# magenta/ddsp

Measured on NVIDIA H100. Metric: audio samples/sec (Harmonic+FilteredNoise decoder), higher is better.
Workload: dtype f32

## Files before the change

### ddsp_b200/csrc/harmonic_v4.cuh

```cuda
#pragma once
#include "harmonic_common.cuh"

namespace ddsp {

__device__ __noinline__ float harmonic_sample_exact(const float* x0,
                                                    const float* x1, float w0,
                                                    float w1, uint32_t p32,
                                                    float f_lo, float f_hi,
                                                    float frac, int K,
                                                    float nyq) {
  float acc = 0.f;
  uint32_t pk = 0;
  for (int k = 1; k <= K; ++k) {
    pk += p32;
    if (!(ref_harmonic_freq(f_lo, f_hi, frac, k) < nyq)) continue;
    float a = x0[k - 1] * w0 + x1[k - 1] * w1;
    acc = fmaf(a, sinpif((float)(int)pk * 4.656612873077393e-10f), acc);
  }
  return acc;
}

namespace hv4 {

constexpr int NW = 4;
constexpr int NT = NW * 32;
constexpr int MIN_CTAS = 6;

#ifdef DDSP_HV4_TIMING
constexpr int kTimingPhases = 8;
__device__ unsigned long long g_hv4_timing[kMaxSMs * (kTimingPhases + 1)];
#define HV4_TIMING_DECL                                                                 \
  unsigned tacc__[kTimingPhases] = {0, 0, 0, 0, 0, 0, 0, 0};                            \
  unsigned tprev__ = (unsigned)clock()
#define HV4_LAP(i)                                                                      \
  do {                                                                                  \
    const unsigned n__ = (unsigned)clock();                                             \
    tacc__[i] += n__ - tprev__;                                                         \
    tprev__ = n__;                                                                      \
  } while (0)
#define HV4_TIMING_FLUSH()                                                              \
  do {                                                                                  \
    if (lane == 0) {                                                                    \
      unsigned smid__;                                                                  \
      asm volatile("mov.u32 %0, %%smid;" : "=r"(smid__));                               \
      unsigned long long* t__ = g_hv4_timing + (smid__ % kMaxSMs) * (kTimingPhases + 1); \
      for (int i__ = 0; i__ < kTimingPhases; ++i__) atomicAdd(t__ + i__, (unsigned long long)tacc__[i__]); \
      atomicAdd(t__ + kTimingPhases, 1ull);                                             \
    }                                                                                   \
  } while (0)
#else
#define HV4_TIMING_DECL
#define HV4_LAP(i)
#define HV4_TIMING_FLUSH()
#endif

struct __align__(16) FrameRec {
  unsigned long long P, A;
  unsigned long long D;
  int ng;
  int rem;
  float f_lo, f_hi, amp0, amp1;
};
static_assert(sizeof(FrameRec) == 48, "FrameRec must be three 16-byte words");

struct Smem {
  size_t off_mbar, off_sin, off_cos, off_x, off_w, off_red, off_inv, off_rec, off_live, total;
};

__host__ __device__ inline Smem smem_layout(int FW, int Kp, int hop) {
  Smem s;
  const size_t FT = (size_t)FW * NW;
  size_t o = 0;
  s.off_mbar = o; o += 16;
  s.off_sin = o;  o += sizeof(float) * kSinTab;
  s.off_cos = o;  o += sizeof(float) * kSinTab;
  s.off_x = o;    o += sizeof(float) * (FT + 1) * Kp;
  s.off_w = o;    o += (hop == 64) ? 0 : sizeof(float) * hop;
  o = (o + 15) & ~(size_t)15;
  s.off_red = o;  o += 16 * NW;
  s.off_rec = o;  o += sizeof(FrameRec) * FT;
  s.off_inv = o;  o += sizeof(float) * (FT + 1);
  s.off_live = o; o += sizeof(int) * (FT + 1);
  s.total = (o + 15) & ~(size_t)15;
  return s;
}

using hcm::phase32;

__device__ __forceinline__ float4 lds128(uint32_t a) {
  float4 v;
  asm volatile("ld.shared.v4.f32 {%0, %1, %2, %3}, [%4];"
               : "=f"(v.x), "=f"(v.y), "=f"(v.z), "=f"(v.w)
               : "r"(a));
  return v;
}

__device__ __forceinline__ float2 bffma2(float x, float2 v, float2 acc) {
  return ffma2(make_float2(x, x), v, acc);
}
__device__ __forceinline__ float2 bfmul2(float x, float2 v) {
  return fmul2(make_float2(x, x), v);
}

__device__ __forceinline__ void controls_rows4(float* __restrict__ sXw,
                                               const int* __restrict__ sLive,
                                               float* __restrict__ sInv, int r0,
                                               int nrows, int Kp, bool raw_scale,
                                               int lane) {
  const int K4 = Kp >> 2;
  const int sub = lane >> 3, l8 = lane & 7;
  const int r = r0 + sub;
  const bool row_ok = r < nrows;
  float4* row4 = reinterpret_cast<float4*>(sXw + (row_ok ? r : r0) * Kp);
  const int live = row_ok ? sLive[r] : 0;
  const int live4 = (live + 3) >> 2;
  float sum = 0.f;
  int c4 = l8;
  for (; c4 < live4; c4 += 8) {
    float4 x = row4[c4];
    if (raw_scale) {
      x.x = exp_sigmoid_f(x.x); x.y = exp_sigmoid_f(x.y);
      x.z = exp_sigmoid_f(x.z); x.w = exp_sigmoid_f(x.w);
    }
    const int k = 4 * c4;
    if (k + 1 >= live) x.y = 0.f;
    if (k + 2 >= live) x.z = 0.f;
    if (k + 3 >= live) x.w = 0.f;
    sum += (x.x + x.y) + (x.z + x.w);
    row4[c4] = x;
  }
  if (row_ok) {
    const float4 z = make_float4(0.f, 0.f, 0.f, 0.f);
    for (; c4 < K4; c4 += 8) row4[c4] = z;
  }
  sum += __shfl_xor_sync(0xffffffffu, sum, 4);
  sum += __shfl_xor_sync(0xffffffffu, sum, 2);
  sum += __shfl_xor_sync(0xffffffffu, sum, 1);
  if (row_ok && l8 == 0) sInv[r] = __fdividef(1.0f, (sum == 0.0f) ? 1e-7f : sum);
}

__device__ __forceinline__ void controls_rows(float* __restrict__ sXw,
                                              const int* __restrict__ sLive, int r0,
                                              int nrows, int Kp, bool raw_scale,
                                              int lane) {
  const int K4 = Kp >> 2;
  const int sub = lane >> 3, l8 = lane & 7;
  const int r = r0 + sub;
  const bool row_ok = r < nrows;
  float4* row4 = reinterpret_cast<float4*>(sXw + (row_ok ? r : r0) * Kp);
  const int live = sLive[row_ok ? r : r0];
  float sum = 0.f;
  if (row_ok) {
    for (int c4 = l8; c4 < K4; c4 += 8) {
      float4 v = make_float4(0.f, 0.f, 0.f, 0.f);
      if (4 * c4 < live) {
        v = row4[c4];
        float e[4] = {v.x, v.y, v.z, v.w};
#pragma unroll
        for (int u = 0; u < 4; ++u) {
          float w = e[u];
          if (raw_scale) w = exp_sigmoid_f(w);
          if (4 * c4 + u >= live) w = 0.f;
          e[u] = w;
          sum += w;
        }
        v = make_float4(e[0], e[1], e[2], e[3]);
      }
      row4[c4] = v;
    }
  }
  sum += __shfl_xor_sync(0xffffffffu, sum, 4);
  sum += __shfl_xor_sync(0xffffffffu, sum, 2);
  sum += __shfl_xor_sync(0xffffffffu, sum, 1);
  const float inv = 1.0f / ((sum == 0.0f) ? 1e-7f : sum);
  if (row_ok) {
    for (int c4 = l8; 4 * c4 < live; c4 += 8) {
      float4 v = row4[c4];
      v.x *= inv; v.y *= inv; v.z *= inv; v.w *= inv;
      row4[c4] = v;
    }
  }
}

__device__ __forceinline__ int row_live_count(float fq, int K, float nyquist, bool nyq) {
  int live = K;
  if (nyq && fq > 0.f) {
    int k = (int)fminf(nyquist / fq, (float)K);
    while (k < K && __fmul_rn(fq, (float)(k + 1)) < nyquist) ++k;
    while (k > 0 && !(__fmul_rn(fq, (float)k) < nyquist)) --k;
    live = k;
  }
  return live;
}

__device__ __noinline__ float sample_exact(const float* x0, int row_stride, float w0,
                                           float w1, uint32_t p32, float f_lo, float f_hi,
                                           float frac, int K, float nyq) {
  return harmonic_sample_exact(x0, x0 + row_stride, w0, w1, p32, f_lo, f_hi, frac, K, nyq);
}

struct Osc2 {
  float2 vo, ve, dlo, dle, na, sg;
  float2 s0e, s0o, s1e, s1o;
  float2 t0e, t0o, t1e, t1o;
};

__device__ __forceinline__ void osc_seed2(Osc2& st, uint32_t qa, uint32_t qb,
                                          const float* __restrict__ sSin,
                                          const float* __restrict__ sCos) {
  const uint32_t ia = qa >> (32 - kSinTabBits), ib = qb >> (32 - kSinTabBits);
  const float2 tx = make_float2(sSin[ia], sSin[ib]);
  const float2 ty = make_float2(sCos[ia], sCos[ib]);
  constexpr uint32_t kLow = (1u << (32 - kSinTabBits)) - 1u;
  constexpr float kC = 1.4629180792671596e-9f;
  constexpr float kOff = -(float)(1u << (31 - kSinTabBits)) * kC;
  const float2 eps = ffma2(make_float2((float)(qa & kLow), (float)(qb & kLow)),
                                make_float2(kC, kC), make_float2(kOff, kOff));
  const float2 e2 = fmul2(eps, eps);
  const float2 ce = ffma2(e2, make_float2(-0.5f, -0.5f), make_float2(1.f, 1.f));
  const float2 se = fmul2(eps, ffma2(e2, make_float2(-0.16666667f, -0.16666667f),
                                               make_float2(1.f, 1.f)));
  const float2 nse = make_float2(-se.x, -se.y);
  const float2 s1 = ffma2(ty, se, fmul2(tx, ce));
  const float2 c1 = ffma2(tx, nse, fmul2(ty, ce));
  const float2 ss = fmul2(s1, s1), cc = fmul2(c1, c1);
  const float2 s2 = fmul2(fadd2(s1, s1), c1);
  st.sg = make_float2(ss.x > cc.x ? -1.0f : 1.0f, ss.y > cc.y ? -1.0f : 1.0f);
  st.na = fmul2(make_float2(fminf(ss.x, cc.x), fminf(ss.y, cc.y)),
                     make_float2(-4.0f, -4.0f));
  st.vo = s1;
  st.ve = s2;
  st.dlo = ffma2(s1, st.sg, s1);
  st.dle = s2;
}

__device__ __forceinline__ void osc_step(Osc2& st) {
  st.dlo = ffma2(st.na, st.vo, st.dlo);
  st.dle = ffma2(st.na, st.ve, st.dle);
  st.vo = fadd2(st.vo, st.dlo);
  st.ve = fadd2(st.ve, st.dle);
}

__device__ __forceinline__ void osc_group(Osc2& st, const float4& X0, const float4& X1) {
  st.s0e = bffma2(X0.x, st.vo, st.s0e);
  st.s1e = bffma2(X1.x, st.vo, st.s1e);
  st.t0e = bffma2(X0.y, st.ve, st.t0e);
  st.t1e = bffma2(X1.y, st.ve, st.t1e);
  osc_step(st);
  st.s0o = bffma2(X0.z, st.vo, st.s0o);
  st.s1o = bffma2(X1.z, st.vo, st.s1o);
  st.t0o = bffma2(X0.w, st.ve, st.t0o);
  st.t1o = bffma2(X1.w, st.ve, st.t1o);
  osc_step(st);
}

__device__ __forceinline__ void osc_group_first(Osc2& st, const float4& X0,
                                                const float4& X1) {
  st.s0e = bfmul2(X0.x, st.vo);
  st.s1e = bfmul2(X1.x, st.vo);
  st.t0e = bfmul2(X0.y, st.ve);
  st.t1e = bfmul2(X1.y, st.ve);
  osc_step(st);
  st.s0o = bfmul2(X0.z, st.vo);
  st.s1o = bfmul2(X1.z, st.vo);
  st.t0o = bfmul2(X0.w, st.ve);
  st.t1o = bfmul2(X1.w, st.ve);
  osc_step(st);
}

__device__ __forceinline__ void osc_group_masked(Osc2& st, const float4& X0,
                                                 const float4& X1, int k, int ka,
                                                 int kb) {
  float2 mo = make_float2(k + 1 <= ka ? st.vo.x : 0.f, k + 1 <= kb ? st.vo.y : 0.f);
  float2 me = make_float2(k + 2 <= ka ? st.ve.x : 0.f, k + 2 <= kb ? st.ve.y : 0.f);
  st.s0e = bffma2(X0.x, mo, st.s0e);
  st.s1e = bffma2(X1.x, mo, st.s1e);
  st.t0e = bffma2(X0.y, me, st.t0e);
  st.t1e = bffma2(X1.y, me, st.t1e);
  osc_step(st);
  mo = make_float2(k + 3 <= ka ? st.vo.x : 0.f, k + 3 <= kb ? st.vo.y : 0.f);
  me = make_float2(k + 4 <= ka ? st.ve.x : 0.f, k + 4 <= kb ? st.ve.y : 0.f);
  st.s0o = bffma2(X0.z, mo, st.s0o);
  st.s1o = bffma2(X1.z, mo, st.s1o);
  st.t0o = bffma2(X0.w, me, st.t0o);
  st.t1o = bffma2(X1.w, me, st.t1o);
  osc_step(st);
}

__device__ __forceinline__ float4 mask4u(const float4& X, int rem) {
  return make_float4(X.x, rem > 1 ? X.y : 0.f, rem > 2 ? X.z : 0.f, 0.f);
}

struct LaneConst {
  uint32_t c1a, c2a, c1b, c2b;
  float2 w1;
};

template <bool WINDOW>
__device__ __forceinline__ LaneConst lane_const(int r0, int lane, float inv_hop,
                                                const float* __restrict__ sW) {
  LaneConst c;
  const uint32_t ra = r0 + lane, rb = ra + 32;
  c.c1a = ra + 1; c.c2a = (ra * (ra + 1)) >> 1;
  c.c1b = rb + 1; c.c2b = (rb * (rb + 1)) >> 1;
  asm volatile("" : "+r"(c.c1a), "+r"(c.c2a), "+r"(c.c1b), "+r"(c.c2b));
  if (sW != nullptr) {
    c.w1 = make_float2(sW[ra], sW[rb]);
  } else {
    const float fa = (float)ra * inv_hop, fb = (float)rb * inv_hop;
    c.w1 = make_float2(WINDOW ? (0.5f - 0.5f * cospif(fa)) : fa,
                       WINDOW ? (0.5f - 0.5f * cospif(fb)) : fb);
  }
  asm volatile("" : "+f"(c.w1.x), "+f"(c.w1.y));
  return c;
}

__device__ __forceinline__ void frame_chunk(
    const float* __restrict__ sX, int xoff, int Kp, const FrameRec* __restrict__ rec,
    const LaneConst& lc, int r0, float inv_hop, const float* __restrict__ sSin,
    const float* __restrict__ sCos, int K, float nyquist, int lane,
    float* __restrict__ out, int accumulate) {
  const float* __restrict__ x0 = sX + xoff;
  const uint32_t kp4 = (uint32_t)Kp << 2;
  const ulonglong2 PA = *reinterpret_cast<const ulonglong2*>(&rec->P);
  const uint4 Dk = *reinterpret_cast<const uint4*>(&rec->D);
  const float4 fa = *reinterpret_cast<const float4*>(&rec->f_lo);
  const unsigned long long D = ((unsigned long long)Dk.y << 32) | Dk.x;
  const int ng = (int)Dk.z, rem = (int)Dk.w;
  const uint32_t qa = phase32(PA.x, PA.y, D, lc.c1a, lc.c2a);
  const uint32_t qb = phase32(PA.x, PA.y, D, lc.c1b, lc.c2b);
  const float2 w0 = ffma2(make_float2(-lc.w1.x, -lc.w1.y), make_float2(fa.z, fa.z),
                               make_float2(fa.z, fa.z));
  const float2 w1 = bfmul2(fa.w, lc.w1);
  float2 y;
  if (ng < 0) {
    constexpr uint32_t kRound = 1u << (31 - kSinTabBits);
    int ra = r0 + lane, xo = xoff;
    asm volatile("" : "+r"(ra), "+r"(xo));
    const float fra = (float)ra * inv_hop, frb = (float)(ra + 32) * inv_hop;
    y.x = sample_exact(sX + xo, Kp, w0.x, w1.x, qa - kRound, fa.x, fa.y, fra, K, nyquist);
    y.y = sample_exact(sX + xo, Kp, w0.y, w1.y, qb - kRound, fa.x, fa.y, frb, K, nyquist);
  } else {
    Osc2 st;
    osc_seed2(st, qa, qb, sSin, sCos);
    if (ng > 0) {
      uint32_t a = smem_u32(x0);
      const uint32_t a_end = a + (ng << 4);
      osc_group_first(st, lds128(a), lds128(a + kp4));
      a += 16;
      if ((ng & 1) == 0) {
        osc_group(st, lds128(a), lds128(a + kp4));
        a += 16;
      }
#pragma unroll 1
      while (a != a_end) {
        osc_group(st, lds128(a), lds128(a + kp4));
        osc_group(st, lds128(a + 16), lds128(a + kp4 + 16));
        a += 32;
      }
      if (rem != 0) osc_group(st, mask4u(lds128(a), rem), mask4u(lds128(a + kp4), rem));
    } else {
      int ra = r0 + lane;
      asm volatile("" : "+r"(ra));
      const float fra = (float)ra * inv_hop, frb = (float)(ra + 32) * inv_hop;
      const int ka = live_harmonics(fa.x, fa.y, fra, K, nyquist);
      const int kb = live_harmonics(fa.x, fa.y, frb, K, nyquist);
      const int kmin = __reduce_min_sync(0xffffffffu, min(ka, kb));
      const int kmax = __reduce_max_sync(0xffffffffu, max(ka, kb));
      st.s0e = st.s0o = st.s1e = st.s1o = make_float2(0.f, 0.f);
      st.t0e = st.t0o = st.t1e = st.t1o = make_float2(0.f, 0.f);
      uint32_t a = smem_u32(x0);
      const uint32_t a_main = a + ((kmin & ~3) << 2);
      if (kmin & 4) {
        osc_group(st, lds128(a), lds128(a + kp4));
        a += 16;
      }
#pragma unroll 1
      while (a != a_main) {
        osc_group(st, lds128(a), lds128(a + kp4));
        osc_group(st, lds128(a + 16), lds128(a + kp4 + 16));
        a += 32;
      }
      for (int k = kmin & ~3; k < kmax; k += 4, a += 16)
        osc_group_masked(st, lds128(a), lds128(a + kp4), k, ka, kb);
    }
    const float2 t0 = ffma2(st.sg, fadd2(st.s0o, st.t0o), fadd2(st.s0e, st.t0e));
    const float2 t1 = ffma2(st.sg, fadd2(st.s1o, st.t1o), fadd2(st.s1e, st.t1e));
    y = ffma2(t1, w1, fmul2(t0, w0));
  }
  if (accumulate) {
    y.x += out[0];
    y.y += out[32];
  }
  out[0] = y.x;
  out[32] = y.y;
}

template <bool WINDOW, int HOPT>
__global__ void __launch_bounds__(NT, MIN_CTAS)
harmonic_v4_kernel(HarmonicParams p, int use_tma, int FW) {
  extern __shared__ __align__(16) unsigned char smem_raw[];
  const int hop = HOPT ? HOPT : p.hop;
  const int Kp = p.Kp, K = p.K, F = p.F;
  const int FT = FW * NW;
  const Smem L = smem_layout(FW, Kp, hop);
  void* mbar = (void*)(smem_raw + L.off_mbar);
  float* sSin = (float*)(smem_raw + L.off_sin);
  float* sCos = (float*)(smem_raw + L.off_cos);
  float* sX = (float*)(smem_raw + L.off_x);
  float* sW = (HOPT == 64) ? nullptr : (float*)(smem_raw + L.off_w);
  double* sRedD = (double*)(smem_raw + L.off_red);
  unsigned long long* sWarpTot = (unsigned long long*)(smem_raw + L.off_red) + NW;
  float* sInv = (float*)(smem_raw + L.off_inv);
  FrameRec* sRec = (FrameRec*)(smem_raw + L.off_rec);
  int* sLive = (int*)(smem_raw + L.off_live);

  const int b = blockIdx.y;
  const int i0 = blockIdx.x * FT;
  const int nfr = min(FT, F - i0);
  const int rows_in = min(nfr + 1, F - i0);
  const int tid = threadIdx.x, lane = tid & 31, warp = tid >> 5;
  const float* f0b = p.f0 + (size_t)b * F;
  const float* ampb = p.amps + (size_t)b * F;

  asm volatile("griddepcontrol.launch_dependents;" ::: "memory");
  HV4_TIMING_DECL;
  if (use_tma && tid == 0) {
    mbar_init(mbar, 1);
    const uint32_t bytes = (uint32_t)rows_in * (uint32_t)K * 4u;
    mbar_expect_tx(mbar, bytes);
    tma_bulk_g2s(sX, p.hd + ((size_t)b * F + i0) * K, bytes, mbar);
  }

  const int n_rec = (FT + 31) >> 5;
  const bool rec_warp = warp < n_rec;
  const int fr = warp * 32 + lane;
  const int cnt = max(0, min(32, nfr - warp * 32));
  const bool raw_scale = p.ctl_flags & DDSP_B200_CTL_SCALE;
  const int n_ctl = (NW > n_rec) ? NW - n_rec : NW;
  const int cw = (NW > n_rec) ? warp - n_rec : warp;
  const int rw = (nfr + n_ctl - 1) / n_ctl;
  const int c0 = cw * rw;
  const int ncr = (cw < 0) ? 0 : max(0, min(rw, nfr - c0));
  const bool c_last = ncr > 0 && c0 + ncr == nfr;
  const int nrows = ncr + ((c_last && rows_in > nfr) ? 1 : 0);
  const float f_row = (lane < nrows) ? f0b[min(i0 + c0 + lane, F - 1)] : 0.f;
  float f = 0.f, a = 0.f, f_tile = 0.f, f_first = 0.f;
  float f_x = 0.f, a_x = 0.f;
  if (rec_warp && cnt > 0) {
    if (lane <= cnt) {
      const int g = min(i0 + fr, F - 1);
      f = f0b[g];
      a = ampb[g];
    }
    if (lane == 31 && cnt == 32) {
      const int g = min(i0 + fr + 1, F - 1);
      f_x = f0b[g];
      a_x = ampb[g];
    }
    f_tile = f0b[i0];
    f_first = f0b[0];
  }
  constexpr int TPT = kSinTab / NT;
  static_assert(TPT * NT == kSinTab, "the table splits evenly over the CTA");
  float2 tab[TPT];
#pragma unroll
  for (int u = 0; u < TPT; ++u) tab[u] = hcm::g_sincos256[tid + u * NT];
  double part = 0.0;
  if ((reinterpret_cast<uintptr_t>(f0b) & 15) == 0) {
    const float4* f4 = reinterpret_cast<const float4*>(f0b);
    const int n4 = i0 >> 2;
    float4 v[4];
    int j = tid;
    for (; j + 3 * NT < n4; j += 4 * NT) {
#pragma unroll
      for (int u = 0; u < 4; ++u) v[u] = f4[j + u * NT];
#pragma unroll
      for (int u = 0; u < 4; ++u)
        part += ((double)v[u].x + (double)v[u].y) + ((double)v[u].z + (double)v[u].w);
    }
#pragma unroll
    for (int u = 0; u < 4; ++u)
      v[u] = (j + u * NT < n4) ? f4[j + u * NT] : make_float4(0.f, 0.f, 0.f, 0.f);
    const float tail = (tid < (i0 & 3)) ? f0b[4 * n4 + tid] : 0.f;
#pragma unroll
    for (int u = 0; u < 4; ++u)
      part += ((double)v[u].x + (double)v[u].y) + ((double)v[u].z + (double)v[u].w);
    part += (double)tail;
  } else {
#pragma unroll 4
    for (int j = tid; j < i0; j += NT) part += (double)f0b[j];
  }
#pragma unroll
  for (int o = 16; o > 0; o >>= 1) part += __shfl_xor_sync(0xffffffffu, part, o);
  if (lane == 0) sRedD[warp] = part;
#pragma unroll
  for (int u = 0; u < TPT; ++u) {
    sSin[tid + u * NT] = tab[u].x;
    sCos[tid + u * NT] = tab[u].y;
  }
  const float inv_hop = 1.0f / (float)hop;
  if (HOPT != 64) {
    for (int r = tid; r < hop; r += NT) {
      const float frac = (float)r * inv_hop;
      sW[r] = WINDOW ? (0.5f - 0.5f * cospif(frac)) : frac;
    }
  }
  if (!use_tma) {
    if (p.hd != nullptr) {
      const float* hdb = p.hd + ((size_t)b * F + i0) * K;
      for (int idx = tid; idx < rows_in * Kp; idx += NT) {
        int r = idx / Kp, c = idx - r * Kp;
        sX[idx] = (c < K) ? hdb[r * K + c] : 0.f;
      }
    } else {
      for (int idx = tid; idx < rows_in * Kp; idx += NT)
        sX[idx] = (idx % Kp == 0) ? 1.0f : 0.f;
    }
  }
  HV4_LAP(0);
  __syncthreads();
  HV4_LAP(1);

  const bool have_ctl = (p.ctl_flags != 0) && (p.hd != nullptr);
  const bool zero_ok = have_ctl && (p.ctl_flags & DDSP_B200_CTL_NYQUIST);
  unsigned long long excl = 0;
  if (rec_warp && cnt > 0) {
    if (raw_scale && lane <= cnt) a = exp_sigmoid_f(a);
    const float f_next = __shfl_down_sync(0xffffffffu, f, 1);
    const float a_next = __shfl_down_sync(0xffffffffu, a, 1);
    float f_n = f_next, a_n = a_next;
    if (lane == 31 && cnt == 32) {
      f_n = f_x;
      a_n = raw_scale ? exp_sigmoid_f(a_x) : a_x;
    }
    unsigned long long tot = 0;
    double a0 = 0.0, dd = 0.0;
    if (lane < cnt) {
      a0 = (double)f * p.inv_sr;
      const double a1 = (double)f_n * p.inv_sr;
      dd = (a1 - a0) * (1.0 / (double)hop);
      tot = frame_total_fix64(a0, a1, hop);
    }
    const unsigned long long incl = warp_scan_frame_totals(tot, lane);
    excl = incl - tot;
    if (lane == 31) sWarpTot[warp] = incl;
    const bool nyq = p.ctl_flags & DDSP_B200_CTL_NYQUIST;
    const int live = row_live_count(f, K, p.nyquist, nyq);
    int live_next = __shfl_down_sync(0xffffffffu, live, 1);
    if (lane == 31 && cnt == 32) live_next = row_live_count(f_n, K, p.nyquist, nyq);
    int ng = -1, rem = 0;
    if (lane < cnt && f >= 1.0f && f_n >= 1.0f) {
      const int kca = live_harmonics(f, f_n, 0.0f, K, p.nyquist);
      const int kcb = live_harmonics(f, f_n, (float)(hop - 1) * inv_hop, K, p.nyquist);
      ng = 0;
      if (kca == kcb) {
        if (zero_ok && live == kca && live_next <= kca) {
          ng = max(1, (kca + 3) >> 2);
        } else {
          ng = kca >> 2;
          rem = kca & 3;
        }
      }
    }
    if (lane < cnt) {
      FrameRec r;
      r.P = 0; r.A = turns_to_fix64(a0); r.D = turns_to_fix64(dd);
      r.ng = ng; r.rem = rem;
      r.f_lo = f; r.f_hi = f_n; r.amp0 = a; r.amp1 = a_n;
      sRec[fr] = r;
    }
    const int n_act = (nfr + 31) >> 5;
    if (n_act > 1) asm volatile("bar.sync 1, %0;" ::"r"(32 * n_act) : "memory");
    HV4_LAP(2);

    double base_sum = 0.0;
#pragma unroll
    for (int w = 0; w < NW; ++w) base_sum += sRedD[w];
    const double a_tile = (double)f_tile * p.inv_sr;
    const double a_first = (double)f_first * p.inv_sr;
    unsigned long long P0 = tile_phase_base(base_sum, a_first, a_tile, hop, p.inv_sr);
    for (int w = 0; w < warp; ++w) P0 += sWarpTot[w];
    if (lane < cnt) {
      const unsigned long long Pf = P0 + excl;
      sRec[fr].P = Pf + 0x80000000ull + (1ull << (63 - kSinTabBits));
    }
  }
  HV4_LAP(3);

  if (ncr > 0) {
    float* sXw = sX + (size_t)c0 * Kp;
    if (have_ctl) {
      const bool nyq = p.ctl_flags & DDSP_B200_CTL_NYQUIST;
      for (int r = lane; r < nrows; r += 32)
        sLive[c0 + r] = row_live_count(r == lane ? f_row : f0b[min(i0 + c0 + r, F - 1)], K,
                                       p.nyquist, nyq);
      __syncwarp();
    }
    if (use_tma) mbar_wait(mbar, 0);
    HV4_LAP(4);
    if (have_ctl) {
      if (Kp <= 128) {
        for (int r0 = 0; r0 < nrows; r0 += 4)
          controls_rows4(sXw, sLive + c0, sInv + c0, r0, nrows, Kp, raw_scale, lane);
      } else {
        for (int r0 = 0; r0 < nrows; r0 += 4)
          controls_rows(sXw, sLive + c0, r0, nrows, Kp, raw_scale, lane);
        for (int r = lane; r < nrows; r += 32) sInv[c0 + r] = 1.0f;
      }
    } else {
      for (int r = lane; r < nrows; r += 32) sInv[c0 + r] = 1.0f;
    }
    if (c_last && rows_in < nfr + 1) {
      __syncwarp();
      for (int c = lane; c < Kp; c += 32) sXw[ncr * Kp + c] = sXw[(ncr - 1) * Kp + c];
      if (lane == 0) sInv[c0 + ncr] = sInv[c0 + ncr - 1];
    }
  }
  HV4_LAP(5);
  __syncthreads();
  HV4_LAP(6);

  const int w0f = warp * FW;
  const int nfw = max(0, min(FW, nfr - w0f));
  if (nfw > 0) {
    FrameRec* rec = sRec + w0f;
    if (lane < nfw) {
      rec[lane].amp0 *= sInv[w0f + lane];
      rec[lane].amp1 *= sInv[w0f + lane + 1];
    }
    __syncwarp();
    float* o = p.audio + (size_t)b * p.N + (size_t)(i0 + w0f) * hop + lane;
    int xoff = w0f * Kp;
    if (HOPT == 64) {
      const LaneConst lc = lane_const<WINDOW>(0, lane, inv_hop, nullptr);
#pragma unroll 1
      for (int li = 0; li < nfw; ++li, ++rec, xoff += Kp, o += 64) {
        frame_chunk(sX, xoff, Kp, rec, lc, 0, inv_hop, sSin, sCos, K, p.nyquist, lane, o,
                    p.accumulate);
      }
    } else {
      for (int li = 0; li < nfw; ++li, ++rec, xoff += Kp) {
        for (int r0 = 0; r0 < hop; r0 += 64, o += 64) {
          const LaneConst lc = lane_const<WINDOW>(r0, lane, inv_hop, sW);
          frame_chunk(sX, xoff, Kp, rec, lc, r0, inv_hop, sSin, sCos, K, p.nyquist, lane, o,
                      p.accumulate);
        }
      }
    }
  }
  HV4_LAP(7);
  HV4_TIMING_FLUSH();
}

}

inline int launch_harmonic_v4(HarmonicParams p, cudaStream_t st) {
  using namespace hv4;
  p.Kp = (p.K + 3) & ~3;
  int FW = 8;
  const long long want_ctas = 8ll * num_sms();
  while (FW > 4 && (long long)p.B * ((p.F + FW * NW - 1) / (FW * NW)) < want_ctas) FW = (FW + 1) >> 1;
  while (FW > 1 && (long long)p.B * ((p.F + FW * NW - 1) / (FW * NW)) < num_sms()) FW = (FW + 1) >> 1;
  FW =std::max(1, std::min(FW, (p.F + NW - 1) / NW));
  while (FW > 1 && smem_layout(FW, p.Kp, p.hop).total > 64 * 1024) FW = (FW + 1) / 2;
  const size_t smem = smem_layout(FW, p.Kp, p.hop).total;
  if (smem > kMaxDynSmem) return 1;
  const int use_tma = (p.hd != nullptr) && (p.K % 4 == 0) &&
                      (((uintptr_t)p.hd & 15) == 0);
  dim3 grid((p.F + FW * NW - 1) / (FW * NW), p.B);
  const bool win = p.amp_method == DDSP_B200_AMP_WINDOW;
  auto kern = p.hop == 64 ? (win ? harmonic_v4_kernel<true, 64> : harmonic_v4_kernel<false, 64>)
                          : (win ? harmonic_v4_kernel<true, 0> : harmonic_v4_kernel<false, 0>);
  int rc = set_smem(kern, smem, "harmonic_forward(v4)");
  if (rc) return rc;
  kern<<<grid, NT, smem, st>>>(p, use_tma, FW);
  DDSP_CHECK_LAUNCH("harmonic_forward(v4)");
  return 0;
}

}
```

Measured before the change: 48.92 billion.

## Interleave sin/cos table and reuse per-row live counts via named barrier

Merges the separate sin and cos shared-memory tables into one interleaved float2 table, so each oscillator seed does one 64-bit load per index instead of two scalar loads. The record-building warps no longer recompute live harmonic counts with shuffles. They wait on a named barrier for the other warps to fill sLive, then read it. The partial-sum loop also breaks early on out-of-range vector slots. The barrier adds a cross-warp dependency that could stall the record warps, and its arrive/sync counts must match exactly.

```diff
diff --git a/ddsp_b200/csrc/harmonic_v4.cuh b/ddsp_b200/csrc/harmonic_v4.cuh
--- a/ddsp_b200/csrc/harmonic_v4.cuh
+++ b/ddsp_b200/csrc/harmonic_v4.cuh
@@ -64,7 +64,7 @@
 static_assert(sizeof(FrameRec) == 48, "FrameRec must be three 16-byte words");
 
 struct Smem {
-  size_t off_mbar, off_sin, off_cos, off_x, off_w, off_red, off_inv, off_rec, off_live, total;
+  size_t off_mbar, off_tab, off_x, off_w, off_red, off_inv, off_rec, off_live, total;
 };
 
 __host__ __device__ inline Smem smem_layout(int FW, int Kp, int hop) {
@@ -72,8 +72,7 @@
   const size_t FT = (size_t)FW * NW;
   size_t o = 0;
   s.off_mbar = o; o += 16;
-  s.off_sin = o;  o += sizeof(float) * kSinTab;
-  s.off_cos = o;  o += sizeof(float) * kSinTab;
+  s.off_tab = o;  o += sizeof(float2) * kSinTab;
   s.off_x = o;    o += sizeof(float) * (FT + 1) * Kp;
   s.off_w = o;    o += (hop == 64) ? 0 : sizeof(float) * hop;
   o = (o + 15) & ~(size_t)15;
@@ -206,11 +205,11 @@
 };
 
 __device__ __forceinline__ void osc_seed2(Osc2& st, uint32_t qa, uint32_t qb,
-                                          const float* __restrict__ sSin,
-                                          const float* __restrict__ sCos) {
+                                          const float2* __restrict__ sTab) {
   const uint32_t ia = qa >> (32 - kSinTabBits), ib = qb >> (32 - kSinTabBits);
-  const float2 tx = make_float2(sSin[ia], sSin[ib]);
-  const float2 ty = make_float2(sCos[ia], sCos[ib]);
+  const float2 ta = sTab[ia], tb = sTab[ib];
+  const float2 tx = make_float2(ta.x, tb.x);
+  const float2 ty = make_float2(ta.y, tb.y);
   constexpr uint32_t kLow = (1u << (32 - kSinTabBits)) - 1u;
   constexpr float kC = 1.4629180792671596e-9f;
   constexpr float kOff = -(float)(1u << (31 - kSinTabBits)) * kC;
@@ -317,9 +316,8 @@
 
 __device__ __forceinline__ void frame_chunk(
     const float* __restrict__ sX, int xoff, int Kp, const FrameRec* __restrict__ rec,
-    const LaneConst& lc, int r0, float inv_hop, const float* __restrict__ sSin,
-    const float* __restrict__ sCos, int K, float nyquist, int lane,
-    float* __restrict__ out, int accumulate) {
+    const LaneConst& lc, int r0, float inv_hop, const float2* __restrict__ sTab, int K,
+    float nyquist, int lane, float* __restrict__ out, int accumulate) {
   const float* __restrict__ x0 = sX + xoff;
   const uint32_t kp4 = (uint32_t)Kp << 2;
   const ulonglong2 PA = *reinterpret_cast<const ulonglong2*>(&rec->P);
@@ -342,7 +340,7 @@
     y.y = sample_exact(sX + xo, Kp, w0.y, w1.y, qb - kRound, fa.x, fa.y, frb, K, nyquist);
   } else {
     Osc2 st;
-    osc_seed2(st, qa, qb, sSin, sCos);
+    osc_seed2(st, qa, qb, sTab);
     if (ng > 0) {
       uint32_t a = smem_u32(x0);
       const uint32_t a_end = a + (ng << 4);
@@ -405,8 +403,7 @@
   const int FT = FW * NW;
   const Smem L = smem_layout(FW, Kp, hop);
   void* mbar = (void*)(smem_raw + L.off_mbar);
-  float* sSin = (float*)(smem_raw + L.off_sin);
-  float* sCos = (float*)(smem_raw + L.off_cos);
+  float2* sTab = (float2*)(smem_raw + L.off_tab);
   float* sX = (float*)(smem_raw + L.off_x);
   float* sW = (HOPT == 64) ? nullptr : (float*)(smem_raw + L.off_w);
   double* sRedD = (double*)(smem_raw + L.off_red);
@@ -484,8 +481,10 @@
       v[u] = (j + u * NT < n4) ? f4[j + u * NT] : make_float4(0.f, 0.f, 0.f, 0.f);
     const float tail = (tid < (i0 & 3)) ? f0b[4 * n4 + tid] : 0.f;
 #pragma unroll
-    for (int u = 0; u < 4; ++u)
+    for (int u = 0; u < 4; ++u) {
+      if (j + u * NT >= n4) break;
       part += ((double)v[u].x + (double)v[u].y) + ((double)v[u].z + (double)v[u].w);
+    }
     part += (double)tail;
   } else {
 #pragma unroll 4
@@ -495,10 +494,7 @@
   for (int o = 16; o > 0; o >>= 1) part += __shfl_xor_sync(0xffffffffu, part, o);
   if (lane == 0) sRedD[warp] = part;
 #pragma unroll
-  for (int u = 0; u < TPT; ++u) {
-    sSin[tid + u * NT] = tab[u].x;
-    sCos[tid + u * NT] = tab[u].y;
-  }
+  for (int u = 0; u < TPT; ++u) sTab[tid + u * NT] = tab[u];
   const float inv_hop = 1.0f / (float)hop;
   if (HOPT != 64) {
     for (int r = tid; r < hop; r += NT) {
@@ -545,21 +541,26 @@
     const unsigned long long incl = warp_scan_frame_totals(tot, lane);
     excl = incl - tot;
     if (lane == 31) sWarpTot[warp] = incl;
-    const bool nyq = p.ctl_flags & DDSP_B200_CTL_NYQUIST;
-    const int live = row_live_count(f, K, p.nyquist, nyq);
-    int live_next = __shfl_down_sync(0xffffffffu, live, 1);
-    if (lane == 31 && cnt == 32) live_next = row_live_count(f_n, K, p.nyquist, nyq);
     int ng = -1, rem = 0;
+    int kc = -1;
     if (lane < cnt && f >= 1.0f && f_n >= 1.0f) {
       const int kca = live_harmonics(f, f_n, 0.0f, K, p.nyquist);
       const int kcb = live_harmonics(f, f_n, (float)(hop - 1) * inv_hop, K, p.nyquist);
       ng = 0;
       if (kca == kcb) {
-        if (zero_ok && live == kca && live_next <= kca) {
-          ng = max(1, (kca + 3) >> 2);
-        } else {
-          ng = kca >> 2;
-          rem = kca & 3;
+        kc = kca;
+        ng = kca >> 2;
+        rem = kca & 3;
+      }
+    }
+    if (zero_ok) {
+      asm volatile("bar.sync 2, %0;" ::"n"(NT) : "memory");
+      if (kc >= 0) {
+        const int live = sLive[fr];
+        const int live_next = (fr + 1 < rows_in) ? sLive[fr + 1] : live;
+        if (live == kc && live_next <= kc) {
+          ng = max(1, (kc + 3) >> 2);
+          rem = 0;
         }
       }
     }
@@ -588,15 +589,16 @@
   }
   HV4_LAP(3);
 
+  if (ncr > 0 && have_ctl) {
+    const bool nyq = p.ctl_flags & DDSP_B200_CTL_NYQUIST;
+    for (int r = lane; r < nrows; r += 32)
+      sLive[c0 + r] = row_live_count(r == lane ? f_row : f0b[min(i0 + c0 + r, F - 1)], K,
+                                     p.nyquist, nyq);
+    __syncwarp();
+  }
+  if (zero_ok && !rec_warp) asm volatile("bar.arrive 2, %0;" ::"n"(NT) : "memory");
   if (ncr > 0) {
     float* sXw = sX + (size_t)c0 * Kp;
-    if (have_ctl) {
-      const bool nyq = p.ctl_flags & DDSP_B200_CTL_NYQUIST;
-      for (int r = lane; r < nrows; r += 32)
-        sLive[c0 + r] = row_live_count(r == lane ? f_row : f0b[min(i0 + c0 + r, F - 1)], K,
-                                       p.nyquist, nyq);
-      __syncwarp();
-    }
     if (use_tma) mbar_wait(mbar, 0);
     HV4_LAP(4);
     if (have_ctl) {
@@ -636,14 +638,14 @@
       const LaneConst lc = lane_const<WINDOW>(0, lane, inv_hop, nullptr);
 #pragma unroll 1
       for (int li = 0; li < nfw; ++li, ++rec, xoff += Kp, o += 64) {
-        frame_chunk(sX, xoff, Kp, rec, lc, 0, inv_hop, sSin, sCos, K, p.nyquist, lane, o,
+        frame_chunk(sX, xoff, Kp, rec, lc, 0, inv_hop, sTab, K, p.nyquist, lane, o,
                     p.accumulate);
       }
     } else {
       for (int li = 0; li < nfw; ++li, ++rec, xoff += Kp) {
         for (int r0 = 0; r0 < hop; r0 += 64, o += 64) {
           const LaneConst lc = lane_const<WINDOW>(r0, lane, inv_hop, sW);
-          frame_chunk(sX, xoff, Kp, rec, lc, r0, inv_hop, sSin, sCos, K, p.nyquist, lane, o,
+          frame_chunk(sX, xoff, Kp, rec, lc, r0, inv_hop, sTab, K, p.nyquist, lane, o,
                       p.accumulate);
         }
       }
```

Result: no change. 49.00 billion, median of 6 (+0.2%).
